# EnyaHermite/SPH3D-GCN

Measured on AMD Instinct MI355X. Metric: point-cloud blocks/sec (fwd+bwd) SPH3D_s3dis 8192-pt, higher is better.
Workload: dtype f32

## Files before the change

### include/sph3d.h

```cpp
#ifndef SPH3D_H
#define SPH3D_H

#include <stddef.h>

#ifdef __cplusplus
extern "C" {
#endif

typedef void* sph3d_stream_t;

enum {
    SPH3D_OK = 0,
    SPH3D_EINVAL = -1,
    SPH3D_EWORKSPACE = -2,
    SPH3D_ELAUNCH = -3,
    SPH3D_EUNSUPPORTED = -4
};

#define SPH3D_ABI_VERSION 2
int sph3d_abi_version(void);
const char* sph3d_last_error(void);
const char* sph3d_build_info(void);


// ... 155 lines not shown
int sph3d_pointwise_gemm_tn(int R, int Cin, int Cout,
                            const float* X, const float* dY, float* dW,
                            void* workspace, size_t workspace_bytes,
                            sph3d_stream_t stream);
size_t sph3d_pointwise_gemm_tn_workspace(int R, int Cin, int Cout);

size_t sph3d_elu_bn_workspace(int R, int C);
int sph3d_elu_bn_forward(int R, int C, const float* y, const float* gamma, const float* beta,
                         float* running_mean, float* running_var, float momentum, float eps, int training,
                         float* out, float* save_mean, float* save_rstd,
                         void* workspace, size_t workspace_bytes, sph3d_stream_t stream);
int sph3d_elu_bn_backward(int R, int C, const float* y, const float* dout, const float* gamma,
                          const float* save_mean, const float* save_rstd, int training,
                          float* dy, float* dgamma, float* dbeta,
                          void* workspace, size_t workspace_bytes, sph3d_stream_t stream);

int sph3d_pointwise_gemm_bnstats_blocks(int R, int Cin, int Cout);
int sph3d_pointwise_gemm_bnstats(int R, int Cin, int Cout, const float* X, const float* W, const float* bias ,
                                 float* Y, float* partial, sph3d_stream_t stream);
int sph3d_elu_bn_forward_partials(int R, int C, int nblk, const float* partial, const float* y, const float* gamma,
                                  const float* beta, float* running_mean, float* running_var, float momentum, float eps,
                                  float* out, float* save_mean, float* save_rstd, sph3d_stream_t stream);

int sph3d_separable_conv3d_fused_supported(int N, int F, int C, int r, int K, int Cout);
int sph3d_separable_conv3d_fused(int B, int N, int M, int F, int C, int r, int K, int Cout, int act,
                                 const int* nn_index, const int* nn_count, const int* bin_index, const float* input,
                                 const float* depthwise_filter, const float* pointwise_weights, const float* bias,
                                 const float* scale, const float* shift, float* output, sph3d_stream_t stream);

int sph3d_separable_conv3d_train_supported(int N, int F, int C, int r, int K, int Cout);
int sph3d_separable_conv3d_train_blocks(int Cout);
int sph3d_separable_conv3d_train(int B, int N, int M, int F, int C, int r, int K, int Cout,
                                 const int* nn_index, const int* nn_count, const int* bin_index, const float* input,
                                 const float* depthwise_filter, const float* pointwise_weights, const float* bias,
                                 float* depthwise_output, float* y, float* partial, sph3d_stream_t stream);
int sph3d_separable_conv3d_ring_failures(void);

int sph3d_pointwise_gemm_skinny_supported(int R, int K1, int K2, int N);
int sph3d_pointwise_gemm_skinny(int R, int K1, int K2, int N, const float* A1, const float* A2, const float* W, const float* bias,
                                float* Y, sph3d_stream_t stream);
size_t sph3d_pointwise_gemm_skinny_tn_workspace(int R, int K1, int K2, int N);
int sph3d_pointwise_gemm_skinny_tn(int R, int K1, int K2, int N, const float* A1, const float* A2, const float* dY, float* dW,
                                   void* workspace, size_t workspace_bytes, sph3d_stream_t stream);

int sph3d_depthwise_conv3d_cat_supported(int F, int Ca, int Cb, int r);
int sph3d_depthwise_conv3d_cat(int B, int N, int M, int F, int Ca, int Cb, int r, int K, const int* nn_index, const int* nn_count,
// ... 24 lines not shown
```

### sph3d_gcn_amd/_lib.py

```python
import ctypes
import os

import torch

_HERE = os.path.dirname(os.path.abspath(__file__))
LIB_PATH = os.environ.get("SPH3D_LIB") or os.path.join(_HERE, "csrc", "libsph3d.so")

_c_int = ctypes.c_int
_c_float = ctypes.c_float
_c_size_t = ctypes.c_size_t
_vp = ctypes.c_void_p

_I, _F, _P, _S = _c_int, _c_float, _vp, _c_size_t
SIGNATURES = {
    "sph3d_abi_version": (_I, []),
    "sph3d_last_error": (ctypes.c_char_p, []),
    "sph3d_build_info": (ctypes.c_char_p, []),
    "sph3d_build_sphere_neighbor": (_I, [_I, _I, _I, _I, _F, _P, _P, _P, _P, _P, _P]),
    "sph3d_build_sphere_neighbor_fixed": (_I, [_I, _I, _I, _I, _F, _P, _P, _P, _P, _P, _P]),
    "sph3d_build_sphere_neighbor_workspace": (_S, [_I, _I, _I]),
    "sph3d_build_sphere_neighbor_ws": (_I, [_I, _I, _I, _I, _F, _P, _P, _P, _P, _P, _P, _S, _P]),
    "sph3d_build_sphere_neighbor_fixed_ws": (_I, [_I, _I, _I, _I, _F, _P, _P, _P, _P, _P, _P, _S, _P]),
    "sph3d_release_stream_scratch": (_I, [_P]),
    "sph3d_release_all_scratch": (_I, []),
# ... 39 lines not shown
    "sph3d_pointwise_gemm_tn": (_I, [_I] * 3 + [_P, _P, _P, _P, _S, _P]),
    "sph3d_elu_bn_workspace": (_S, [_I] * 2),
    "sph3d_pointwise_gemm_bnstats_blocks": (_I, [_I] * 3),
    "sph3d_pointwise_gemm_bnstats": (_I, [_I] * 3 + [_P] * 6),
    "sph3d_nngrid_launches": (ctypes.c_longlong, []),
    "sph3d_masked_softmax_xent_parts": (_I, [_I]),
    "sph3d_masked_softmax_xent": (_I, [_I, _I, _I] + [_P] * 5 + [_P]),
    "sph3d_adam_step": (_I, [ctypes.c_longlong] + [_P] * 4 + [_F] * 4 + [_I, _P]),
    "sph3d_feed_assemble": (_I, [_I, _I, _I, ctypes.c_longlong, _P, _P, _P, ctypes.c_ulonglong, ctypes.c_ulonglong, _I] + [_P] * 5),
    "sph3d_pointwise_gemm_skinny_supported": (_I, [_I] * 4),
    "sph3d_pointwise_gemm_skinny": (_I, [_I] * 4 + [_P] * 6),
    "sph3d_pointwise_gemm_skinny_tn_workspace": (_S, [_I] * 4),
    "sph3d_pointwise_gemm_skinny_tn": (_I, [_I] * 4 + [_P] * 5 + [_S, _P]),
    "sph3d_separable_conv3d_fused_supported": (_I, [_I] * 6),
    "sph3d_separable_conv3d_fused": (_I, [_I] * 9 + [_P] * 11),
    "sph3d_separable_conv3d_train_supported": (_I, [_I] * 6),
    "sph3d_separable_conv3d_train_blocks": (_I, [_I]),
    "sph3d_separable_conv3d_train": (_I, [_I] * 8 + [_P] * 11),
    "sph3d_separable_conv3d_ring_failures": (_I, []),
    "sph3d_pointwise_gemm_exchange_failures": (_I, []),
    "sph3d_elu_bn_forward_partials": (_I, [_I] * 3 + [_P] * 6 + [_F, _F] + [_P] * 4),
    "sph3d_elu_bn_forward": (_I, [_I, _I, _P, _P, _P, _P, _P, _F, _F, _I, _P, _P, _P, _P, _S, _P]),
    "sph3d_elu_bn_backward": (_I, [_I, _I] + [_P] * 5 + [_I] + [_P] * 3 + [_P, _S, _P]),
}
_EXTRA = {
    "sph3d_selftest_math": (_I, [_I, _P, _P, _P, _P, _P, _P, _P]),
}

ABI_VERSION = 2
_lib = None


class Sph3dError(RuntimeError):
    pass


def lib():
    global _lib
    if _lib is not None:
        return _lib
    if not os.path.exists(LIB_PATH):
        raise Sph3dError(
            "libsph3d.so is not built (%s).  Run `python -c 'import __graft_entry__ as g; g.build()'` "
            "or `make -C sph3d_gcn_amd/csrc`.  There is no fallback path." % LIB_PATH)
    l = ctypes.CDLL(LIB_PATH)
    for table in (SIGNATURES, _EXTRA):
# ... 118 lines not shown
def ptr(t):
    return t.data_ptr() if t is not None else None


_scratch = {}


def release_scratch(stream=None):
    for key in [k for k in _scratch if stream is None or k[1] == stream]:
        del _scratch[key]


def scratch(nbytes, device, slot=0):
    if not nbytes:
        return None
    key = (device.index, current_raw_stream(), slot)
    t = _scratch.get(key)
    if t is None or t.numel() < nbytes:
        t = torch.empty((nbytes + nbytes // 4,), dtype=torch.uint8, device=device)
        _scratch[key] = t
    return t


class Arena:
    __slots__ = ("device", "cap", "off", "need", "_i32", "_f32", "buf")

    def __init__(self, nbytes, device):
        self.device, self.cap, self.off, self.need = device, int(nbytes), 0, 0
        self.buf = torch.empty((self.cap,), dtype=torch.uint8, device=device) if self.cap > 0 else None
        self._i32 = self.buf.view(torch.int32) if self.buf is not None else None
        self._f32 = self.buf.view(torch.float32) if self.buf is not None else None

    def take(self, shape, dtype):
        n = 4
        for d in shape:
            n *= d
        n = (n + 255) & ~255
        self.need += n
        if n == 0 or self.buf is None or self.off + n > self.cap:
            return None
        base = self._i32 if dtype is torch.int32 else self._f32
        strides, s = [], 1
        for d in reversed(shape):
            strides.append(s)
            s *= d
        strides.reverse()
# ... 33 lines not shown
```

### sph3d_gcn_amd/csrc/gemm.hip

```cpp
#include <atomic>
#include "common.hpp"

namespace sph3d {

typedef float f32x16 __attribute__((ext_vector_type(16)));
typedef float f32x4 __attribute__((ext_vector_type(4)));
typedef float f32x2 __attribute__((ext_vector_type(2)));
__device__ __forceinline__ f32x4 as_v4(const float4 v) { f32x4 r; r.x = v.x; r.y = v.y; r.z = v.z; r.w = v.w; return r; }

constexpr int BM = 128;
constexpr int BKS = 16;
constexpr int BKL = 32;

__device__ __forceinline__ float4 load4_guard(const float* __restrict__ p, int ld, int r, int c, int rows, int cols, bool vec_ok)
{
    float4 v = make_float4(0.f, 0.f, 0.f, 0.f);
    if (r < rows) {
        const float* q = p + (size_t)r * ld + c;
        if (vec_ok && c + 3 < cols) {
            v = *reinterpret_cast<const float4*>(q);
        } else {
            if (c < cols) v.x = q[0];
            if (c + 1 < cols) v.y = q[1];
            if (c + 2 < cols) v.z = q[2];
// ... 119 lines not shown
    __device__ __forceinline__ void issue(const float* __restrict__ base, float* image) const
    {
        const int wave = __builtin_amdgcn_readfirstlane((int)threadIdx.x >> 6);
#pragma unroll
        for (int i = 0; i < NI; i++) {
            __builtin_amdgcn_global_load_lds((const __attribute__((address_space(1))) void*)(base + voff[i]),
                                             (__attribute__((address_space(3))) void*)(image + (wave * NI + i) * 256), 16, 0, 0);
        }
    }
    static __device__ __forceinline__ f32x4 frag(const float* image, int row, int g, int lk)
    {
        if (KM) return *reinterpret_cast<const f32x4*>(image + ((row << 2) + ((2 * g + lk) ^ ((row >> 2) & 3))) * 4);
        const float* q = image + (8 * g + 4 * lk) * BT + (row ^ (lk << 5));
        return f32x4{q[0], q[BT], q[2 * BT], q[3 * BT]};
    }
};

constexpr int kDmaWgs = 5;
constexpr int cmax_i(int a, int b) { return a > b ? a : b; }

template <int BMT, int BN, int TM, int TN, bool SPLITK, bool GUARD, bool STATS, bool EPX, int LDSF>
__device__ __forceinline__ void gemm_epilogue(f32x16 (&acc)[TM][TN], float* lds, int M, int N, float* __restrict__ Cmat, int ldc,
                                              const float* __restrict__ bias, int act, float* __restrict__ stats, int tm, int ksplit,
                                              int m0, int n0, int wave, int lane, int wm, int wn, int li, int lk)
{
    constexpr int WN = BN / 2;
    float* Cout = SPLITK ? Cmat + (size_t)ksplit * ((size_t)M * ldc) : Cmat;
    if (!GUARD) {
        constexpr int EP = EPX ? WN : WN + 4;
        static_assert(4 * 32 * EP <= LDSF, "epilogue staging must fit the operand LDS");
        float* stage = lds + wave * (32 * EP);
        constexpr int LPR = WN / 4;
        constexpr int RPI = 64 / LPR;
        if constexpr (STATS) {
#pragma unroll
            for (int j = 0; j < TN; j++) {
                const float bv = bias != nullptr ? bias[n0 + wn + j * 32 + li] : 0.f;
                float sz = 0.f, sq = 0.f;
#pragma unroll
                for (int i = 0; i < TM; i++)
#pragma unroll
                    for (int e = 0; e < 16; e++) {
                        const float y = acc[i][j][e] + bv;
                        const float z = y > 0.f ? y : __expf(y) - 1.f;
                        sz += z;
                        sq = fmaf(z, z, sq);
                    }
                sz += __shfl_xor(sz, 32);
                sq += __shfl_xor(sq, 32);
                if (lk == 0) {
                    float* sp = stats + (size_t)(tm * 2 + (wave >> 1)) * 2 * N + n0 + wn + j * 32 + li;
                    sp[0] = sz;
                    sp[N] = sq;
                }
            }
        }
#pragma unroll
        for (int i = 0; i < TM; i++) {
#pragma unroll
            for (int j = 0; j < TN; j++) {
                const int col = wn + j * 32 + li;
                const float bv = (!SPLITK && bias != nullptr) ? bias[n0 + col] : 0.f;
#pragma unroll
                for (int e = 0; e < 16; e++) {
                    float v = acc[i][j][e] + bv;
                    if (!SPLITK && act == 1) v = v > 0.f ? v : expm1f(v);
                    stage[((e & 3) + 8 * (e >> 2) + 4 * lk) * EP + ((j * 32 + li) ^ (EPX ? (lk << 5) : 0))] = v;
                }
            }
#pragma unroll
            for (int it = 0; it < 32 / RPI; it++) {
                const int r = it * RPI + lane / LPR;
                const int c4 = (lane % LPR) * 4;
                const float4 v = *reinterpret_cast<const float4*>(&stage[r * EP + (c4 ^ (EPX ? (((r >> 2) & 1) << 5) : 0))]);
                *reinterpret_cast<float4*>(&Cout[(size_t)(m0 + wm + i * 32 + r) * ldc + n0 + wn + c4]) = v;
            }
        }
        return;
    }
#pragma unroll
    for (int i = 0; i < TM; i++) {
#pragma unroll
        for (int j = 0; j < TN; j++) {
            const int col = n0 + wn + j * 32 + li;
            const float bv = (!SPLITK && bias != nullptr && col < N) ? bias[col] : 0.f;
#pragma unroll
            for (int e = 0; e < 16; e++) {
                const int row = m0 + wm + i * 32 + (e & 3) + 8 * (e >> 2) + 4 * lk;
                if (row < M && col < N) {
                    float v = acc[i][j][e] + bv;
                    if (!SPLITK && act == 1) v = v > 0.f ? v : expm1f(v);
                    Cout[(size_t)row * ldc + col] = v;
                }
            }
        }
    }
}

template <bool AK, bool BKM, int BMT, int BN, int BK, bool SPLITK, bool GUARD, bool STATS = false>
__global__ __launch_bounds__(256, (BK == 16 && !GUARD) ? kDmaWgs : 2) void gemm_f32_mfma(int M, int N, int Kd, const float* __restrict__ A, int lda,
                                                     const float* __restrict__ B, int ldb, float* __restrict__ Cmat,
                                                     int ldc, const float* __restrict__ bias, int act, int kchunk,
                                                     float* __restrict__ stats = nullptr, int nsplit = 1)
{
    using SA = Stage<AK, BMT, BK>;
    using SB = Stage<BKM, BN, BK>;
    constexpr int LDK = BK + 4;
    constexpr bool DMA = !GUARD && BK == 16;
    constexpr int WM = BMT / 2, WN = BN / 2;
    constexpr int LDSF = DMA ? cmax_i(2 * (BMT + BN) * BK, 4 * 32 * (WN == 64 ? WN : WN + 4)) : 2 * (SA::LDS_FLOATS + SB::LDS_FLOATS);
    __shared__ __attribute__((aligned(16))) float lds[LDSF];
    constexpr int TM = WM / 32, TN = WN / 32;

    const int tiles_n = (N + BN - 1) / BN;
    const int tiles_m = (M + BMT - 1) / BMT;
    const int wg = (int)blockIdx.x;
    int tm, tn, ksplit = 0;
    if (SPLITK) {
        const int T = tiles_m * tiles_n;
        const int g = wg / (8 * T), r = wg - g * 8 * T;
        ksplit = g * 8 + (r & 7);
        if (ksplit >= nsplit) return;
        const int tile = r >> 3;
        tm = tile / tiles_n;
        tn = tile - tm * tiles_n;
    } else {
// ... 119 lines not shown
            for (int s4 = 0; s4 < 4; s4++) {
#pragma unroll
                for (int i = 0; i < TM; i++)
#pragma unroll
                    for (int j = 0; j < TN; j++) {
                        const float av = s4 == 0 ? af[i].x : (s4 == 1 ? af[i].y : (s4 == 2 ? af[i].z : af[i].w));
                        const float bv = s4 == 0 ? bf[j].x : (s4 == 1 ? bf[j].y : (s4 == 2 ? bf[j].z : bf[j].w));
                        acc[i][j] = __builtin_amdgcn_mfma_f32_32x32x2f32(av, bv, acc[i][j], 0, 0, 0);
                    }
            }
        }
        __builtin_amdgcn_s_setprio(0);
        if (more) {
            sa.store(lds + (buf ^ 1) * BUF);
            sb.store(lds + (buf ^ 1) * BUF + SA::LDS_FLOATS);
        }
        __syncthreads();
        buf ^= 1;
    }

    }

    gemm_epilogue<BMT, BN, TM, TN, SPLITK, GUARD, STATS, DMA && WN == 64, LDSF>(acc, lds, M, N, Cmat, ldc, bias, act, stats, tm, ksplit,
                                                                                  m0, n0, wave, lane, wm, wn, li, lk);
}

typedef __bf16 bf16x8 __attribute__((ext_vector_type(8)));
typedef unsigned u32x2v __attribute__((ext_vector_type(2)));

struct Split3 { unsigned h, m, l; };
__device__ __forceinline__ Split3 split_pair(float a, float b)
{
    Split3 r;
    const unsigned ua = __float_as_uint(a), ub = __float_as_uint(b);
    r.h = __builtin_amdgcn_perm(ub, ua, 0x07060302u);
    const float ra = a - __uint_as_float(ua & 0xffff0000u), rb = b - __uint_as_float(ub & 0xffff0000u);
    const unsigned va = __float_as_uint(ra), vb = __float_as_uint(rb);
    r.m = __builtin_amdgcn_perm(vb, va, 0x07060302u);
    const float sa = ra - __uint_as_float(va & 0xffff0000u), sb = rb - __uint_as_float(vb & 0xffff0000u);
    r.l = __builtin_amdgcn_perm(__float_as_uint(sb), __float_as_uint(sa), 0x07060302u);
    return r;
}

template <bool KMAJ, int BT, int BK>
struct SplitStage {
    static constexpr int KG = BK / 8;
    static constexpr int PLANE = KG * BT * 16;
// ... 65 lines not shown
                for (int j = 0; j < 4; j++) {
                    const Split3 sp = split_pair(a[j], b[j]);
                    char* q = img + (slot(k0 >> 3, rq * 4 + j) << 4) + ((k0 & 7) << 1);
                    *reinterpret_cast<unsigned*>(q) = sp.h;
                    *reinterpret_cast<unsigned*>(q + PLANE) = sp.m;
                    *reinterpret_cast<unsigned*>(q + 2 * PLANE) = sp.l;
                }
            }
        }
    }
    __device__ __forceinline__ static bf16x8 frag(const char* img, int pc, int row, int g)
    {
        return *reinterpret_cast<const bf16x8*>(img + pc * PLANE + (slot(g, row) << 4));
    }
};

__device__ int g_xs_fail = 0;

template <bool AK, bool BKM, int BMT, int BN, int BK, bool SPLITK, bool STATS, bool GUARD = false, bool XS = false>
__global__ __launch_bounds__(256, 4) void gemm_split_mfma(int M, int N, int Kd, const float* __restrict__ A, int lda,
                                                          const float* __restrict__ B, int ldb, float* __restrict__ Cmat, int ldc,
                                                          const float* __restrict__ bias, int act, int kchunk,
                                                          float* __restrict__ stats = nullptr, int nsplit = 1,
                                                          float* __restrict__ xslab = nullptr, int* __restrict__ xflag = nullptr)
{
    static_assert(!(XS && SPLITK) && !(XS && GUARD), "the exchange variant is an unguarded, non-slab kernel");
    using PA = SplitStage<AK, BMT, BK>;
    using PB = SplitStage<BKM, BN, BK>;
    constexpr int WM = BMT / 2, WN = BN / 2;
    constexpr int TM = WM / 32, TN = WN / 32;
    constexpr int BUFB = PA::BYTES + PB::BYTES;
    constexpr bool EPX = WN == 64;
    constexpr int LDSF = cmax_i(BUFB / 4, 4 * 32 * (EPX ? WN : WN + 4));
    __shared__ __attribute__((aligned(16))) float lds[LDSF];
    char* img = reinterpret_cast<char*>(lds);

    const int tiles_n = (N + BN - 1) / BN;
    const int tiles_m = (M + BMT - 1) / BMT;
    const int wg = (int)blockIdx.x;
    int tm, tn, ksplit = 0;
    if (XS) {
        const int Tg = ((tiles_m + 7) / 8) * 8 * tiles_n;
        const int rev = wg / Tg, wl = wg - rev * Tg;
        ksplit = nsplit - 1 - rev;
        const int g = wl / (8 * tiles_n), r = wl - g * 8 * tiles_n;
        tm = g * 8 + (r & 7);
        tn = r >> 3;
// ... 115 lines not shown
            int polls = 0;
            while (__hip_atomic_load(&xflag[tile], __ATOMIC_RELAXED, __HIP_MEMORY_SCOPE_AGENT) < nsplit - 1) {
                __builtin_amdgcn_s_sleep(4);
                if (++polls > (1 << 20)) {
                    atomicAdd(&g_xs_fail, 1);
                    break;
                }
            }
            __hip_atomic_store(&xflag[tile], 0, __ATOMIC_RELAXED, __HIP_MEMORY_SCOPE_AGENT);
        }
        __syncthreads();
        for (int ks = 1; ks < nsplit; ks++) {
            const float* sl = xslab + ((size_t)(ks - 1) * ntile + tile) * (NW * 256) + threadIdx.x;
#pragma unroll
            for (int i = 0; i < TM; i++)
#pragma unroll
                for (int j = 0; j < TN; j++)
#pragma unroll
                    for (int e = 0; e < 16; e++)
                        acc[i][j][e] += __hip_atomic_load(&sl[((i * TN + j) * 16 + e) * 256], __ATOMIC_RELAXED, __HIP_MEMORY_SCOPE_AGENT);
        }
    }
    gemm_epilogue<BMT, BN, TM, TN, SPLITK, GUARD, STATS, EPX, LDSF>(acc, lds, M, N, Cmat, ldc, bias, act, stats, tm, ksplit, m0, n0, wave,
                                                                      lane, wm, wn, li, lk);
}

__global__ __launch_bounds__(256) void gemm_reduce_splits(int nsplit, int total, const float* __restrict__ partial,
                                                          float* __restrict__ out)
{
    __shared__ float red[8][32];
    const int cx = (int)threadIdx.x & 31, py = (int)threadIdx.x >> 5;
    const int j = blockIdx.x * 32 + cx;
    float s = 0.f;
    if (j < total) {
        for (int p0 = py; p0 < nsplit; p0 += 64) {
            float v[8];
#pragma unroll
            for (int u = 0; u < 8; u++) {
                const int p = p0 + u * 8;
                v[u] = partial[(size_t)(p < nsplit ? p : py) * total + j];
            }
#pragma unroll
            for (int u = 0; u < 8; u++)
                if (p0 + u * 8 < nsplit) s += v[u];
        }
    }
    red[py][cx] = s;
// ... 144 lines not shown
extern "C" int sph3d_pointwise_gemm_mode(int mode)
{
    if (mode == 0 || mode == 1) return g_split_mode.exchange(mode);
    return g_split_mode.load();
}

extern "C" int sph3d_pointwise_gemm(int R, int Cin, int Cout, const float* X, const float* W, const float* bias, int act,
                                    int trans_w, float* Y, sph3d_stream_t stream)
{
    SPH3D_REQUIRE(R >= 0 && Cin > 0 && Cout > 0, "pointwise_gemm: bad dims R=%d Cin=%d Cout=%d", R, Cin, Cout);
    SPH3D_REQUIRE(act == 0 || act == 1, "pointwise_gemm: act must be 0 (none) or 1 (ELU), got %d", act);
    if (R == 0) return SPH3D_OK;
    hipStream_t st = as_stream(stream);
    if (trans_w) return launch_gemm<true, true>(R, Cout, Cin, X, Cin, W, Cin, Y, Cout, bias, act, st);
    return launch_gemm<true, false>(R, Cout, Cin, X, Cin, W, Cout, Y, Cout, bias, act, st);
}

extern "C" int sph3d_pointwise_gemm_bnstats_blocks(int R, int Cin, int Cout)
{
    int bm = 0, bn = 0;
    return (R > 0 && Cin > 0 && Cout > 0) ? nn_stats_tile(R, Cout, Cin, bm, bn) : 0;
}

extern "C" int sph3d_pointwise_gemm_bnstats(int R, int Cin, int Cout, const float* X, const float* W, const float* bias, float* Y,
                                            float* partial, sph3d_stream_t stream)
{
    SPH3D_REQUIRE(R > 0 && Cin > 0 && Cout > 0, "pointwise_gemm_bnstats: bad dims R=%d Cin=%d Cout=%d", R, Cin, Cout);
    int bm = 0, bn = 0;
    const int nblk = nn_stats_tile(R, Cout, Cin, bm, bn);
    if (nblk == 0 || !aligned16(X) || !aligned16(W) || !aligned16(Y)) {
        set_error("pointwise_gemm_bnstats: shape (%d, %d -> %d) needs whole tiles and 16-byte aligned operands", R, Cin, Cout);
        return SPH3D_EUNSUPPORTED;
    }
    hipStream_t st = as_stream(stream);
    const unsigned tiles = gemm_grid(R / bm, Cout / bn);
    if (split_on()) {
        if (bm == 128 && bn == 128)
            hipLaunchKernelGGL((gemm_split_mfma<true, false, 128, 128, 16, false, true>), dim3(tiles), dim3(256), 0, st, R, Cout, Cin, X, Cin, W,
                               Cout, Y, Cout, bias, 0, 0, partial);
        else if (bm == 128)
            hipLaunchKernelGGL((gemm_split_mfma<true, false, 128, 64, 16, false, true>), dim3(tiles), dim3(256), 0, st, R, Cout, Cin, X, Cin, W,
                               Cout, Y, Cout, bias, 0, 0, partial);
        else if (Cin % 32 == 0) {
            const int ns = xs_splits(tiles, Cin, 32, kXsCap);
            char* xb = ns > 1 ? xs_buffer(st, (long long)(R / 64) * (Cout / 64), ns, 64 * 64) : nullptr;
            if (xb != nullptr)
                hipLaunchKernelGGL((gemm_split_mfma<true, false, 64, 64, 32, false, true, false, true>), dim3(tiles * ns), dim3(256), 0, st, R, Cout,
                                   Cin, X, Cin, W, Cout, Y, Cout, bias, 0, Cin / ns, partial, ns, (float*)(xb + kXsFlagBytes), (int*)xb);
            else
                hipLaunchKernelGGL((gemm_split_mfma<true, false, 64, 64, 32, false, true>), dim3(tiles), dim3(256), 0, st, R, Cout, Cin, X, Cin, W,
                                   Cout, Y, Cout, bias, 0, 0, partial);
        } else
            hipLaunchKernelGGL((gemm_split_mfma<true, false, 64, 64, 16, false, true>), dim3(tiles), dim3(256), 0, st, R, Cout, Cin, X, Cin, W,
                               Cout, Y, Cout, bias, 0, 0, partial);
        return check_launch("sph3d_pointwise_gemm_bnstats");
    }
    if (bm == 128 && bn == 128)
        hipLaunchKernelGGL((gemm_f32_mfma<true, false, 128, 128, BKS, false, false, true>), dim3(tiles), dim3(256), 0, st, R, Cout, Cin, X,
                           Cin, W, Cout, Y, Cout, bias, 0, 0, partial);
    else if (bm == 128)
        hipLaunchKernelGGL((gemm_f32_mfma<true, false, 128, 64, BKS, false, false, true>), dim3(tiles), dim3(256), 0, st, R, Cout, Cin, X,
                           Cin, W, Cout, Y, Cout, bias, 0, 0, partial);
    else
        hipLaunchKernelGGL((gemm_f32_mfma<true, false, 64, 64, BKS, false, false, true>), dim3(tiles), dim3(256), 0, st, R, Cout, Cin, X,
                           Cin, W, Cout, Y, Cout, bias, 0, 0, partial);
    return check_launch("sph3d_pointwise_gemm_bnstats");
}

extern "C" size_t sph3d_pointwise_gemm_tn_workspace(int R, int Cin, int Cout)
{
    int bn, tiles, nsplit, kchunk;
    tn_plan(R, Cin, Cout, bn, tiles, nsplit, kchunk);
    return nsplit > 1 ? sizeof(float) * (size_t)nsplit * Cin * Cout : 0;
}

extern "C" int sph3d_pointwise_gemm_tn(int R, int Cin, int Cout, const float* X, const float* dY, float* dW,
                                       void* workspace, size_t workspace_bytes, sph3d_stream_t stream)
{
    SPH3D_REQUIRE(R > 0 && Cin > 0 && Cout > 0, "pointwise_gemm_tn: bad dims R=%d Cin=%d Cout=%d", R, Cin, Cout);
    hipStream_t st = as_stream(stream);
    int bn, tiles, nsplit, kchunk;
    tn_plan(R, Cin, Cout, bn, tiles, nsplit, kchunk);
    const size_t need = sph3d_pointwise_gemm_tn_workspace(R, Cin, Cout);
    if (need > 0 && (workspace == nullptr || workspace_bytes < need)) {
        set_error("pointwise_gemm_tn: workspace %zu B < required %zu B", workspace_bytes, need);
        return SPH3D_EWORKSPACE;
    }
    float* out = nsplit > 1 ? (float*)workspace : dW;
    const bool whole = (Cin % 128 == 0) && (Cout % bn == 0) && (R % kchunk == 0) && aligned16(X) && aligned16(dY) && aligned16(out);
// ... 44 lines not shown
```

### sph3d_gcn_amd/csrc/norm.hip

```cpp
#include "common.hpp"

namespace sph3d {

constexpr int kNormMaxBlocks = 1024;

__device__ __forceinline__ float elu1(float y) { return y > 0.f ? y : __expf(y) - 1.f; }

template <bool BWD>
__global__ __launch_bounds__(256) void norm_reduce_kernel(int R, int C, const float* __restrict__ y,
                                                          const float* __restrict__ dout, const float* __restrict__ mean,
                                                          const float* __restrict__ rstd, float* __restrict__ partial)
{
    __shared__ float4 red[2][256];
    const int cg = C >> 2;
    const int rows_per_iter = 256 / cg > 0 ? 256 / cg : 1;
    const int tx = (int)threadIdx.x % cg, ty = (int)threadIdx.x / cg;
    const bool act = ty < rows_per_iter;
    const int rows_per_block = (R + (int)gridDim.x - 1) / (int)gridDim.x;
    const int r0 = (int)blockIdx.x * rows_per_block;
    const int r1 = (r0 + rows_per_block) < R ? (r0 + rows_per_block) : R;
    float4 a = make_float4(0.f, 0.f, 0.f, 0.f), b = a;
    float4 mu = a, rs = a;
    if (BWD && act) {
        mu = *reinterpret_cast<const float4*>(&mean[tx * 4]);
// ... 146 lines not shown
            o.y = fmaf((elu1(v.y) - mu.y) * rs.y, ga.y, be.y);
            o.z = fmaf((elu1(v.z) - mu.z) * rs.z, ga.z, be.z);
            o.w = fmaf((elu1(v.w) - mu.w) * rs.w, ga.w, be.w);
        } else {
            const float4 g = reinterpret_cast<const float4*>(dout)[i];
            const float4 c0 = *reinterpret_cast<const float4*>(&coef[c]);
            const float4 c1 = *reinterpret_cast<const float4*>(&coef[C + c]);
#define SPH3D_BN_BWD(e)                                                             \
    {                                                                               \
        const float z = elu1(v.e);                                                  \
        const float zh = (z - mu.e) * rs.e;                                         \
        const float dz = ga.e * rs.e * (g.e - c0.e - zh * c1.e);                    \
        o.e = v.e > 0.f ? dz : dz * (z + 1.f);                                      \
    }
            SPH3D_BN_BWD(x) SPH3D_BN_BWD(y) SPH3D_BN_BWD(z) SPH3D_BN_BWD(w)
#undef SPH3D_BN_BWD
        }
        reinterpret_cast<float4*>(out)[i] = o;
    }
}

static int norm_blocks(int R) { int b = (R + 31) / 32; return b < 1 ? 1 : (b > kNormMaxBlocks ? kNormMaxBlocks : b); }

}

using namespace sph3d;

extern "C" size_t sph3d_elu_bn_workspace(int R, int C)
{
    return sizeof(float) * ((size_t)norm_blocks(R) * 2 * C + 2 * (size_t)C);
}

extern "C" int sph3d_elu_bn_forward(int R, int C, const float* y, const float* gamma, const float* beta,
                                    float* running_mean, float* running_var, float momentum, float eps, int training,
                                    float* out, float* save_mean, float* save_rstd,
                                    void* workspace, size_t workspace_bytes, sph3d_stream_t stream)
{
    SPH3D_REQUIRE(R > 0 && C > 0 && C % 4 == 0 && C <= 1024, "elu_bn: needs R>0, C%%4==0, C<=1024 (got R=%d C=%d)", R, C);
    const size_t need = sph3d_elu_bn_workspace(R, C);
    if (workspace == nullptr || workspace_bytes < need) {
        set_error("elu_bn_forward: workspace %zu B < required %zu B", workspace_bytes, need);
        return SPH3D_EWORKSPACE;
    }
    hipStream_t st = as_stream(stream);
    float* partial = (float*)workspace;
    const int nblk = norm_blocks(R);
// ... 35 lines not shown
                                     const float* save_mean, const float* save_rstd, int training,
                                     float* dy, float* dgamma, float* dbeta,
                                     void* workspace, size_t workspace_bytes, sph3d_stream_t stream)
{
    SPH3D_REQUIRE(R > 0 && C > 0 && C % 4 == 0 && C <= 1024, "elu_bn: needs R>0, C%%4==0, C<=1024 (got R=%d C=%d)", R, C);
    const size_t need = sph3d_elu_bn_workspace(R, C);
    if (workspace == nullptr || workspace_bytes < need) {
        set_error("elu_bn_backward: workspace %zu B < required %zu B", workspace_bytes, need);
        return SPH3D_EWORKSPACE;
    }
    hipStream_t st = as_stream(stream);
    float* partial = (float*)workspace;
    const int nblk = norm_blocks(R);
    float* coef = partial + (size_t)nblk * 2 * C;
    hipLaunchKernelGGL(norm_reduce_kernel<true>, dim3(nblk), dim3(256), 0, st, R, C, y, dout, save_mean, save_rstd, partial);
    hipLaunchKernelGGL(norm_bwd_finalize, dim3((C + 31) / 32), dim3(32 * kFinLanes), 0, st, R, C, nblk, training, partial, dgamma, dbeta, coef);
    const long long total4 = (long long)R * C / 4;
    long long blocks = (total4 + 255) / 256;
    if (blocks > 4096) blocks = 4096;
    hipLaunchKernelGGL(norm_apply_kernel<true>, dim3((unsigned)blocks), dim3(256), 0, st, total4, C, y, dout, save_mean,
                       save_rstd, gamma, nullptr, coef, dy);
    return check_launch("sph3d_elu_bn_backward");
}
```

### sph3d_gcn_amd/tf_norm.py

```python
from typing import Optional, Tuple

import torch

from . import _lib

MOMENTUM = 0.99
EPSILON = 1e-3


def supported(C):
    return C % 4 == 0 and C <= 1024


def _fwd_impl(y: torch.Tensor, gamma: torch.Tensor, beta: torch.Tensor, moving_mean: torch.Tensor,
              moving_var: torch.Tensor, training: bool) -> Tuple[torch.Tensor, torch.Tensor, torch.Tensor]:
    _lib.require_device(y, gamma, beta, moving_mean, moving_var)
    y = _lib.f32(y)
    C = y.shape[-1]
    R = y.numel() // C
    out = torch.empty_like(y)
    save_mean = torch.empty((C,), dtype=torch.float32, device=y.device)
    save_rstd = torch.empty((C,), dtype=torch.float32, device=y.device)
    l = _lib.lib()
    wsb = l.sph3d_elu_bn_workspace(R, C)
# ... 89 lines not shown
    save_rstd = torch.empty((C,), dtype=torch.float32, device=y.device)
    _lib.check(_lib.lib().sph3d_elu_bn_forward_partials(R, C, partial.shape[0], _lib.ptr(partial), _lib.ptr(y), _lib.ptr(gamma),
                                                         _lib.ptr(beta), _lib.ptr(moving_mean), _lib.ptr(moving_var),
                                                         1.0 - MOMENTUM, EPSILON, _lib.ptr(out), _lib.ptr(save_mean),
                                                         _lib.ptr(save_rstd), _lib.stream_ptr()))
    return out, save_mean, save_rstd


_gemm_bnstats = torch.library.custom_op("sph3d::pointwise_gemm_bnstats", mutates_args=())(_gemm_bnstats_impl)
_elu_bn_partials = torch.library.custom_op("sph3d::elu_bn_partials", mutates_args=("moving_mean", "moving_var"))(_elu_bn_partials_impl)


@_gemm_bnstats.register_fake
def _(x, w, bias=None):
    nblk = gemm_bn_blocks(x.shape[0], x.shape[1], w.shape[1])
    return x.new_empty((x.shape[0], w.shape[1])), x.new_empty((nblk, 2, w.shape[1]))


@_elu_bn_partials.register_fake
def _(y, partial, gamma, beta, moving_mean, moving_var):
    return torch.empty_like(y), torch.empty_like(gamma), torch.empty_like(gamma)


class _GemmEluBnFn(torch.autograd.Function):

    @staticmethod
    def forward(ctx, x, w, bias, gamma, beta, moving_mean, moving_var):
        y, partial = _gemm_bnstats_impl(x, w, bias)
        out, save_mean, save_rstd = _elu_bn_partials_impl(y, partial, gamma, beta, moving_mean, moving_var)
        ctx.save_for_backward(x, w, y, gamma, save_mean, save_rstd)
        ctx.has_bias = bias is not None
        return out

    @staticmethod
    def backward(ctx, dout):
        from . import tf_gemm
        x, w, y, gamma, save_mean, save_rstd = ctx.saved_tensors
        dy, dgamma, dbeta = _bwd_impl(y, dout, gamma, save_mean, save_rstd, True)
        dx = tf_gemm._pointwise_gemm_impl(dy, w, True) if ctx.needs_input_grad[0] else None
        dw = tf_gemm._pointwise_gemm_tn_impl(x, dy) if ctx.needs_input_grad[1] else None
        db = dy.sum(0) if (ctx.has_bias and ctx.needs_input_grad[2]) else None
        return dx, dw, db, dgamma, dbeta, None, None


def gemm_elu_batch_norm(x, w, gamma, beta, moving_mean, moving_var, bias=None):
    return _GemmEluBnFn.apply(x, w, bias, gamma, beta, moving_mean, moving_var)
```

Baseline: 2059.

## Fold batch-norm statistics finalize into GEMM tail via last-block reduction

Adds a last-arriving-workgroup tail to the pointwise GEMM+BN-stats kernel. Workgroups count arrivals with atomic counters, the final block of each row group reduces the per-tile partials in double, and a final group computes mean, rstd and the running stats. This removes the separate stats-reduction pass that the old partials-based forward launched. The apply step is now a lightweight separate kernel. In exchange it adds atomic counters, persistent zeroed scratch and a serialized tail inside the GEMM, with a fallback launch when there are few blocks.

```diff
diff --git a/include/sph3d.h b/include/sph3d.h
--- a/include/sph3d.h
+++ b/include/sph3d.h
@@ -201,6 +201,15 @@
                                   const float* beta, float* running_mean, float* running_var, float momentum, float eps,
                                   float* out, float* save_mean, float* save_rstd, sph3d_stream_t stream);
 
+size_t sph3d_pointwise_gemm_bnstats_tail_workspace(int R, int Cin, int Cout);
+size_t sph3d_pointwise_gemm_bnstats_tail_counters_workspace(void);
+int sph3d_pointwise_gemm_bnstats_tail(int R, int Cin, int Cout, const float* X, const float* W, const float* bias ,
+                                      float* Y, float* running_mean, float* running_var, float momentum, float eps,
+                                      float* save_mean, float* save_rstd, void* workspace, size_t workspace_bytes,
+                                      void* counters, sph3d_stream_t stream);
+int sph3d_elu_bn_apply(int R, int C, const float* y, const float* gamma, const float* beta, const float* save_mean,
+                       const float* save_rstd, float* out, sph3d_stream_t stream);
+
 int sph3d_separable_conv3d_fused_supported(int N, int F, int C, int r, int K, int Cout);
 int sph3d_separable_conv3d_fused(int B, int N, int M, int F, int C, int r, int K, int Cout, int act,
                                  const int* nn_index, const int* nn_count, const int* bin_index, const float* input,
diff --git a/sph3d_gcn_amd/_lib.py b/sph3d_gcn_amd/_lib.py
--- a/sph3d_gcn_amd/_lib.py
+++ b/sph3d_gcn_amd/_lib.py
@@ -85,6 +85,10 @@
     "sph3d_elu_bn_forward_partials": (_I, [_I] * 3 + [_P] * 6 + [_F, _F] + [_P] * 4),
     "sph3d_elu_bn_forward": (_I, [_I, _I, _P, _P, _P, _P, _P, _F, _F, _I, _P, _P, _P, _P, _S, _P]),
     "sph3d_elu_bn_backward": (_I, [_I, _I] + [_P] * 5 + [_I] + [_P] * 3 + [_P, _S, _P]),
+    "sph3d_pointwise_gemm_bnstats_tail_counters_workspace": (_S, []),
+    "sph3d_elu_bn_apply": (_I, [_I, _I] + [_P] * 7),
+    "sph3d_pointwise_gemm_bnstats_tail_workspace": (_S, [_I] * 3),
+    "sph3d_pointwise_gemm_bnstats_tail": (_I, [_I] * 3 + [_P] * 6 + [_F, _F] + [_P] * 3 + [_S, _P, _P]),
 }
 _EXTRA = {
     "sph3d_selftest_math": (_I, [_I, _P, _P, _P, _P, _P, _P, _P]),
@@ -249,6 +253,15 @@
     return t
 
 
+def zeroed_scratch(nbytes, device, slot):
+    key = (device.index, current_raw_stream(), slot)
+    t = _scratch.get(key)
+    if t is None or t.numel() < nbytes:
+        t = torch.zeros((nbytes,), dtype=torch.uint8, device=device)
+        _scratch[key] = t
+    return t
+
+
 class Arena:
     __slots__ = ("device", "cap", "off", "need", "_i32", "_f32", "buf")
 
diff --git a/sph3d_gcn_amd/csrc/bn_tail.hpp b/sph3d_gcn_amd/csrc/bn_tail.hpp
--- /dev/null
+++ b/sph3d_gcn_amd/csrc/bn_tail.hpp
@@ -0,0 +1,140 @@
+#pragma once
+#include <hip/hip_runtime.h>
+
+namespace sph3d {
+
+constexpr int kBnTailMaxGroups = 64;
+constexpr int kBnTailCounterWords = 128;
+constexpr int kBnTailLdsBytes = 16 + 2 * 256 * 8;
+
+struct BnTail {
+    unsigned* cnt = nullptr;
+    double* gsum = nullptr;
+    int rpg = 0;
+    int R = 0;
+    float* o0 = nullptr;
+    float* o1 = nullptr;
+    float* o2 = nullptr;
+    float* o3 = nullptr;
+    float eps = 0.f, momentum = 0.f;
+    int training = 1;
+};
+
+constexpr int kBnTailMinRows = 1024;
+void launch_norm_fwd_finalize(int R, int C, int nblk, const float* partial, float eps, float momentum, float* mean, float* rstd,
+                              float* run_mean, float* run_var, hipStream_t st);
+
+static inline int bn_tail_rows_per_group(int nrows)
+{
+    if (nrows <= 64) return nrows;
+    const int need = ((nrows + kBnTailMaxGroups - 1) / kBnTailMaxGroups + 1) & ~1;
+    return need > 32 ? need : 32;
+}
+static inline int bn_tail_groups(int nrows) { const int g = bn_tail_rows_per_group(nrows); return (nrows + g - 1) / g; }
+
+__device__ __forceinline__ void bn_tail_store(float* p, float v) { __hip_atomic_store(p, v, __ATOMIC_RELAXED, __HIP_MEMORY_SCOPE_AGENT); }
+
+__device__ __forceinline__ bool bn_tail_last(unsigned* cnt, unsigned expect, unsigned* flag)
+{
+    asm volatile("s_waitcnt vmcnt(0)" ::: "memory");
+    __syncthreads();
+    if (threadIdx.x == 0) {
+        const unsigned t = __hip_atomic_fetch_add(cnt, 1u, __ATOMIC_RELAXED, __HIP_MEMORY_SCOPE_AGENT);
+        const bool last = t == expect - 1;
+        if (last) __hip_atomic_store(cnt, 0u, __ATOMIC_RELAXED, __HIP_MEMORY_SCOPE_AGENT);
+        *flag = last ? 1u : 0u;
+    }
+    __syncthreads();
+    const bool last = *flag != 0u;
+    __builtin_amdgcn_fence(__ATOMIC_ACQUIRE, "wavefront");
+    return last;
+}
+
+template <typename T>
+__device__ __forceinline__ void bn_tail_fold(const T* src, int C, int k0, int k1, int cb, double* red, double& s, double& q, bool& own)
+{
+    const int tid = (int)threadIdx.x;
+    const int P = C >= 256 ? 1 : 256 / C;
+    const int c = cb + (C >= 256 ? tid : tid % C);
+    const int p = C >= 256 ? 0 : tid / C;
+    const bool act = c < C && p < P;
+    s = 0.0; q = 0.0;
+    if (act) {
+        constexpr int UN = 8;
+        for (int kb = k0 + p; kb < k1; kb += UN * P) {
+            T a[UN], b[UN];
+#pragma unroll
+            for (int u = 0; u < UN; u++) {
+                const int k = kb + u * P;
+                const int kc = k < k1 ? k : kb;
+                a[u] = __hip_atomic_load(&src[(size_t)kc * 2 * C + c], __ATOMIC_RELAXED, __HIP_MEMORY_SCOPE_AGENT);
+                b[u] = __hip_atomic_load(&src[(size_t)kc * 2 * C + C + c], __ATOMIC_RELAXED, __HIP_MEMORY_SCOPE_AGENT);
+            }
+#pragma unroll
+            for (int u = 0; u < UN; u++)
+                if (kb + u * P < k1) { s += (double)a[u]; q += (double)b[u]; }
+        }
+    }
+    red[tid] = s;
+    red[256 + tid] = q;
+    __syncthreads();
+    own = act && p == 0;
+    if (own)
+        for (int j = 1; j < P; j++) { s += red[j * C + (c - cb)]; q += red[256 + j * C + (c - cb)]; }
+    __syncthreads();
+}
+
+template <bool BWD>
+__device__ __forceinline__ void bn_tail_outputs(const BnTail& t, int C, int c, double s, double q)
+{
+    if (!BWD) {
+        const double m = s / t.R;
+        double var = q / t.R - m * m;
+        if (var < 0.0) var = 0.0;
+        t.o0[c] = (float)m;
+        t.o1[c] = (float)(1.0 / sqrt(var + (double)t.eps));
+        if (t.o2 != nullptr) {
+            t.o2[c] = (float)((1.0 - t.momentum) * t.o2[c] + t.momentum * m);
+            t.o3[c] = (float)((1.0 - t.momentum) * t.o3[c] + t.momentum * var);
+        }
+    } else {
+        t.o0[c] = (float)s;
+        t.o1[c] = (float)q;
+        t.o2[c] = t.training ? (float)(s / t.R) : 0.f;
+        t.o2[C + c] = t.training ? (float)(q / t.R) : 0.f;
+    }
+}
+
+template <bool BWD>
+__device__ __forceinline__ void bn_tail_finish(const BnTail& t, const float* partial, int C, int nrows, int group, int arrivals, void* lds)
+{
+    unsigned* flag = reinterpret_cast<unsigned*>(lds);
+    double* red = reinterpret_cast<double*>(reinterpret_cast<char*>(lds) + 16);
+    if (!bn_tail_last(&t.cnt[1 + group], (unsigned)arrivals, flag)) return;
+    const int ngroups = (nrows + t.rpg - 1) / t.rpg;
+    const int k0 = group * t.rpg;
+    const int k1 = (k0 + t.rpg) < nrows ? (k0 + t.rpg) : nrows;
+    for (int cb = 0; cb < C; cb += 256) {
+        double s, q;
+        bool own;
+        bn_tail_fold<float>(partial, C, k0, k1, cb, red, s, q, own);
+        if (own) {
+            const int c = cb + (C >= 256 ? (int)threadIdx.x : (int)threadIdx.x % C);
+            if (ngroups == 1) bn_tail_outputs<BWD>(t, C, c, s, q);
+            else {
+                __hip_atomic_store(&t.gsum[(size_t)group * 2 * C + c], s, __ATOMIC_RELAXED, __HIP_MEMORY_SCOPE_AGENT);
+                __hip_atomic_store(&t.gsum[(size_t)group * 2 * C + C + c], q, __ATOMIC_RELAXED, __HIP_MEMORY_SCOPE_AGENT);
+            }
+        }
+    }
+    if (ngroups == 1) return;
+    if (!bn_tail_last(&t.cnt[0], (unsigned)ngroups, flag)) return;
+    for (int cb = 0; cb < C; cb += 256) {
+        double s, q;
+        bool own;
+        bn_tail_fold<double>(t.gsum, C, 0, ngroups, cb, red, s, q, own);
+        if (own) bn_tail_outputs<BWD>(t, C, cb + (C >= 256 ? (int)threadIdx.x : (int)threadIdx.x % C), s, q);
+    }
+}
+
+}
diff --git a/sph3d_gcn_amd/csrc/gemm.hip b/sph3d_gcn_amd/csrc/gemm.hip
--- a/sph3d_gcn_amd/csrc/gemm.hip
+++ b/sph3d_gcn_amd/csrc/gemm.hip
@@ -1,5 +1,6 @@
 #include <atomic>
 #include "common.hpp"
+#include "bn_tail.hpp"
 
 namespace sph3d {
 
@@ -165,7 +166,7 @@
 template <int BMT, int BN, int TM, int TN, bool SPLITK, bool GUARD, bool STATS, bool EPX, int LDSF>
 __device__ __forceinline__ void gemm_epilogue(f32x16 (&acc)[TM][TN], float* lds, int M, int N, float* __restrict__ Cmat, int ldc,
                                               const float* __restrict__ bias, int act, float* __restrict__ stats, int tm, int ksplit,
-                                              int m0, int n0, int wave, int lane, int wm, int wn, int li, int lk)
+                                              int m0, int n0, int wave, int lane, int wm, int wn, int li, int lk, const BnTail& fin)
 {
     constexpr int WN = BN / 2;
     float* Cout = SPLITK ? Cmat + (size_t)ksplit * ((size_t)M * ldc) : Cmat;
@@ -193,8 +194,13 @@
                 sq += __shfl_xor(sq, 32);
                 if (lk == 0) {
                     float* sp = stats + (size_t)(tm * 2 + (wave >> 1)) * 2 * N + n0 + wn + j * 32 + li;
-                    sp[0] = sz;
-                    sp[N] = sq;
+                    if (fin.cnt == nullptr) {
+                        sp[0] = sz;
+                        sp[N] = sq;
+                    } else {
+                        bn_tail_store(sp, sz);
+                        bn_tail_store(sp + N, sq);
+                    }
                 }
             }
         }
@@ -217,6 +223,15 @@
                 const int c4 = (lane % LPR) * 4;
                 const float4 v = *reinterpret_cast<const float4*>(&stage[r * EP + (c4 ^ (EPX ? (((r >> 2) & 1) << 5) : 0))]);
                 *reinterpret_cast<float4*>(&Cout[(size_t)(m0 + wm + i * 32 + r) * ldc + n0 + wn + c4]) = v;
+            }
+        }
+        if constexpr (STATS) {
+            if (fin.cnt != nullptr) {
+                static_assert(LDSF * 4 >= kBnTailLdsBytes, "the finish borrows the operand LDS");
+                const int tiles_m = M / BMT, tiles_n = N / BN;
+                const int tpg = fin.rpg >> 1, group = tm / tpg;
+                const int t1 = (group + 1) * tpg < tiles_m ? (group + 1) * tpg : tiles_m;
+                bn_tail_finish<false>(fin, stats, N, 2 * tiles_m, group, (t1 - group * tpg) * tiles_n, lds);
             }
         }
         return;
@@ -244,7 +259,7 @@
 __global__ __launch_bounds__(256, (BK == 16 && !GUARD) ? kDmaWgs : 2) void gemm_f32_mfma(int M, int N, int Kd, const float* __restrict__ A, int lda,
                                                      const float* __restrict__ B, int ldb, float* __restrict__ Cmat,
                                                      int ldc, const float* __restrict__ bias, int act, int kchunk,
-                                                     float* __restrict__ stats = nullptr, int nsplit = 1)
+                                                     float* __restrict__ stats = nullptr, int nsplit = 1, BnTail fin = {})
 {
     using SA = Stage<AK, BMT, BK>;
     using SB = Stage<BKM, BN, BK>;
@@ -410,7 +425,7 @@
     }
 
     gemm_epilogue<BMT, BN, TM, TN, SPLITK, GUARD, STATS, DMA && WN == 64, LDSF>(acc, lds, M, N, Cmat, ldc, bias, act, stats, tm, ksplit,
-                                                                                  m0, n0, wave, lane, wm, wn, li, lk);
+                                                                                  m0, n0, wave, lane, wm, wn, li, lk, fin);
 }
 
 typedef __bf16 bf16x8 __attribute__((ext_vector_type(8)));
@@ -522,7 +537,8 @@
                                                           const float* __restrict__ B, int ldb, float* __restrict__ Cmat, int ldc,
                                                           const float* __restrict__ bias, int act, int kchunk,
                                                           float* __restrict__ stats = nullptr, int nsplit = 1,
-                                                          float* __restrict__ xslab = nullptr, int* __restrict__ xflag = nullptr)
+                                                          float* __restrict__ xslab = nullptr, int* __restrict__ xflag = nullptr,
+                                                          BnTail fin = {})
 {
     static_assert(!(XS && SPLITK) && !(XS && GUARD), "the exchange variant is an unguarded, non-slab kernel");
     using PA = SplitStage<AK, BMT, BK>;
@@ -684,7 +700,7 @@
         }
     }
     gemm_epilogue<BMT, BN, TM, TN, SPLITK, GUARD, STATS, EPX, LDSF>(acc, lds, M, N, Cmat, ldc, bias, act, stats, tm, ksplit, m0, n0, wave,
-                                                                      lane, wm, wn, li, lk);
+                                                                      lane, wm, wn, li, lk, fin);
 }
 
 __global__ __launch_bounds__(256) void gemm_reduce_splits(int nsplit, int total, const float* __restrict__ partial,
@@ -875,49 +891,96 @@
     return (R > 0 && Cin > 0 && Cout > 0) ? nn_stats_tile(R, Cout, Cin, bm, bn) : 0;
 }
 
-extern "C" int sph3d_pointwise_gemm_bnstats(int R, int Cin, int Cout, const float* X, const float* W, const float* bias, float* Y,
-                                            float* partial, sph3d_stream_t stream)
-{
-    SPH3D_REQUIRE(R > 0 && Cin > 0 && Cout > 0, "pointwise_gemm_bnstats: bad dims R=%d Cin=%d Cout=%d", R, Cin, Cout);
+static int launch_bnstats(const char* what, int R, int Cin, int Cout, const float* X, const float* W, const float* bias, float* Y,
+                          float* partial, BnTail fin, hipStream_t st)
+{
     int bm = 0, bn = 0;
     const int nblk = nn_stats_tile(R, Cout, Cin, bm, bn);
     if (nblk == 0 || !aligned16(X) || !aligned16(W) || !aligned16(Y)) {
-        set_error("pointwise_gemm_bnstats: shape (%d, %d -> %d) needs whole tiles and 16-byte aligned operands", R, Cin, Cout);
+        set_error("%s: shape (%d, %d -> %d) needs whole tiles and 16-byte aligned operands", what, R, Cin, Cout);
         return SPH3D_EUNSUPPORTED;
     }
-    hipStream_t st = as_stream(stream);
+    float* const nof = nullptr;
+    int* const noi = nullptr;
     const unsigned tiles = gemm_grid(R / bm, Cout / bn);
     if (split_on()) {
         if (bm == 128 && bn == 128)
             hipLaunchKernelGGL((gemm_split_mfma<true, false, 128, 128, 16, false, true>), dim3(tiles), dim3(256), 0, st, R, Cout, Cin, X, Cin, W,
-                               Cout, Y, Cout, bias, 0, 0, partial);
+                               Cout, Y, Cout, bias, 0, 0, partial, 1, nof, noi, fin);
         else if (bm == 128)
             hipLaunchKernelGGL((gemm_split_mfma<true, false, 128, 64, 16, false, true>), dim3(tiles), dim3(256), 0, st, R, Cout, Cin, X, Cin, W,
-                               Cout, Y, Cout, bias, 0, 0, partial);
+                               Cout, Y, Cout, bias, 0, 0, partial, 1, nof, noi, fin);
         else if (Cin % 32 == 0) {
             const int ns = xs_splits(tiles, Cin, 32, kXsCap);
             char* xb = ns > 1 ? xs_buffer(st, (long long)(R / 64) * (Cout / 64), ns, 64 * 64) : nullptr;
             if (xb != nullptr)
                 hipLaunchKernelGGL((gemm_split_mfma<true, false, 64, 64, 32, false, true, false, true>), dim3(tiles * ns), dim3(256), 0, st, R, Cout,
-                                   Cin, X, Cin, W, Cout, Y, Cout, bias, 0, Cin / ns, partial, ns, (float*)(xb + kXsFlagBytes), (int*)xb);
+                                   Cin, X, Cin, W, Cout, Y, Cout, bias, 0, Cin / ns, partial, ns, (float*)(xb + kXsFlagBytes), (int*)xb, fin);
             else
                 hipLaunchKernelGGL((gemm_split_mfma<true, false, 64, 64, 32, false, true>), dim3(tiles), dim3(256), 0, st, R, Cout, Cin, X, Cin, W,
-                                   Cout, Y, Cout, bias, 0, 0, partial);
+                                   Cout, Y, Cout, bias, 0, 0, partial, 1, nof, noi, fin);
         } else
             hipLaunchKernelGGL((gemm_split_mfma<true, false, 64, 64, 16, false, true>), dim3(tiles), dim3(256), 0, st, R, Cout, Cin, X, Cin, W,
-                               Cout, Y, Cout, bias, 0, 0, partial);
-        return check_launch("sph3d_pointwise_gemm_bnstats");
+                               Cout, Y, Cout, bias, 0, 0, partial, 1, nof, noi, fin);
+        return check_launch(what);
     }
     if (bm == 128 && bn == 128)
         hipLaunchKernelGGL((gemm_f32_mfma<true, false, 128, 128, BKS, false, false, true>), dim3(tiles), dim3(256), 0, st, R, Cout, Cin, X,
-                           Cin, W, Cout, Y, Cout, bias, 0, 0, partial);
+                           Cin, W, Cout, Y, Cout, bias, 0, 0, partial, 1, fin);
     else if (bm == 128)
         hipLaunchKernelGGL((gemm_f32_mfma<true, false, 128, 64, BKS, false, false, true>), dim3(tiles), dim3(256), 0, st, R, Cout, Cin, X,
-                           Cin, W, Cout, Y, Cout, bias, 0, 0, partial);
+                           Cin, W, Cout, Y, Cout, bias, 0, 0, partial, 1, fin);
     else
         hipLaunchKernelGGL((gemm_f32_mfma<true, false, 64, 64, BKS, false, false, true>), dim3(tiles), dim3(256), 0, st, R, Cout, Cin, X,
-                           Cin, W, Cout, Y, Cout, bias, 0, 0, partial);
-    return check_launch("sph3d_pointwise_gemm_bnstats");
+                           Cin, W, Cout, Y, Cout, bias, 0, 0, partial, 1, fin);
+    return check_launch(what);
+}
+
+extern "C" int sph3d_pointwise_gemm_bnstats(int R, int Cin, int Cout, const float* X, const float* W, const float* bias, float* Y,
+                                            float* partial, sph3d_stream_t stream)
+{
+    SPH3D_REQUIRE(R > 0 && Cin > 0 && Cout > 0, "pointwise_gemm_bnstats: bad dims R=%d Cin=%d Cout=%d", R, Cin, Cout);
+    return launch_bnstats("sph3d_pointwise_gemm_bnstats", R, Cin, Cout, X, W, bias, Y, partial, BnTail{}, as_stream(stream));
+}
+
+static size_t bnstats_partial_bytes(int nblk, int Cout) { return (sizeof(float) * (size_t)nblk * 2 * Cout + 7) & ~(size_t)7; }
+
+extern "C" size_t sph3d_pointwise_gemm_bnstats_tail_workspace(int R, int Cin, int Cout)
+{
+    const int nblk = sph3d_pointwise_gemm_bnstats_blocks(R, Cin, Cout);
+    if (nblk == 0) return 0;
+    return bnstats_partial_bytes(nblk, Cout) + sizeof(double) * (size_t)bn_tail_groups(nblk) * 2 * Cout;
+}
+
+extern "C" size_t sph3d_pointwise_gemm_bnstats_tail_counters_workspace(void) { return sizeof(unsigned) * kBnTailCounterWords; }
+
+extern "C" int sph3d_pointwise_gemm_bnstats_tail(int R, int Cin, int Cout, const float* X, const float* W, const float* bias, float* Y,
+                                                 float* running_mean, float* running_var, float momentum, float eps,
+                                                 float* save_mean, float* save_rstd, void* workspace, size_t workspace_bytes,
+                                                 void* counters, sph3d_stream_t stream)
+{
+    SPH3D_REQUIRE(R > 0 && Cin > 0 && Cout > 0 && Cout <= 1024, "pointwise_gemm_bnstats_tail: bad dims R=%d Cin=%d Cout=%d", R, Cin, Cout);
+    const int nblk = sph3d_pointwise_gemm_bnstats_blocks(R, Cin, Cout);
+    const size_t need = sph3d_pointwise_gemm_bnstats_tail_workspace(R, Cin, Cout);
+    if (nblk > 0 && (workspace == nullptr || workspace_bytes < need || counters == nullptr)) {
+        set_error("pointwise_gemm_bnstats_tail: workspace %zu B < required %zu B, or no counters", workspace_bytes, need);
+        return SPH3D_EWORKSPACE;
+    }
+    hipStream_t st = as_stream(stream);
+    if (nblk < kBnTailMinRows) {
+        const int rc = launch_bnstats("sph3d_pointwise_gemm_bnstats_tail", R, Cin, Cout, X, W, bias, Y, (float*)workspace, BnTail{}, st);
+        if (rc != SPH3D_OK) return rc;
+        launch_norm_fwd_finalize(R, Cout, nblk, (const float*)workspace, eps, momentum, save_mean, save_rstd, running_mean, running_var, st);
+        return check_launch("sph3d_pointwise_gemm_bnstats_tail");
+    }
+    BnTail t;
+    t.cnt = (unsigned*)counters;
+    t.gsum = (double*)((char*)workspace + bnstats_partial_bytes(nblk, Cout));
+    t.rpg = bn_tail_rows_per_group(nblk);
+    t.R = R;
+    t.o0 = save_mean; t.o1 = save_rstd; t.o2 = running_mean; t.o3 = running_var;
+    t.eps = eps; t.momentum = momentum;
+    return launch_bnstats("sph3d_pointwise_gemm_bnstats_tail", R, Cin, Cout, X, W, bias, Y, (float*)workspace, t, st);
 }
 
 extern "C" size_t sph3d_pointwise_gemm_tn_workspace(int R, int Cin, int Cout)
diff --git a/sph3d_gcn_amd/csrc/norm.hip b/sph3d_gcn_amd/csrc/norm.hip
--- a/sph3d_gcn_amd/csrc/norm.hip
+++ b/sph3d_gcn_amd/csrc/norm.hip
@@ -1,4 +1,5 @@
 #include "common.hpp"
+#include "bn_tail.hpp"
 
 namespace sph3d {
 
@@ -192,6 +193,13 @@
 
 static int norm_blocks(int R) { int b = (R + 31) / 32; return b < 1 ? 1 : (b > kNormMaxBlocks ? kNormMaxBlocks : b); }
 
+void launch_norm_fwd_finalize(int R, int C, int nblk, const float* partial, float eps, float momentum, float* mean, float* rstd,
+                              float* run_mean, float* run_var, hipStream_t st)
+{
+    hipLaunchKernelGGL(norm_fwd_finalize, dim3((C + 31) / 32), dim3(32 * kFinLanes), 0, st, R, C, nblk, partial, eps, momentum, mean, rstd,
+                       run_mean, run_var);
+}
+
 }
 
 using namespace sph3d;
@@ -273,3 +281,15 @@
                        save_rstd, gamma, nullptr, coef, dy);
     return check_launch("sph3d_elu_bn_backward");
 }
+
+extern "C" int sph3d_elu_bn_apply(int R, int C, const float* y, const float* gamma, const float* beta, const float* save_mean,
+                                  const float* save_rstd, float* out, sph3d_stream_t stream)
+{
+    SPH3D_REQUIRE(R > 0 && C > 0 && C % 4 == 0 && C <= 1024, "elu_bn_apply: needs R>0, C%%4==0, C<=1024 (got R=%d C=%d)", R, C);
+    const long long total4 = (long long)R * C / 4;
+    long long blocks = (total4 + 255) / 256;
+    if (blocks > 4096) blocks = 4096;
+    hipLaunchKernelGGL(norm_apply_kernel<false>, dim3((unsigned)blocks), dim3(256), 0, as_stream(stream), total4, C, y, nullptr, save_mean,
+                       save_rstd, gamma, beta, nullptr, out);
+    return check_launch("sph3d_elu_bn_apply");
+}
diff --git a/sph3d_gcn_amd/tf_norm.py b/sph3d_gcn_amd/tf_norm.py
--- a/sph3d_gcn_amd/tf_norm.py
+++ b/sph3d_gcn_amd/tf_norm.py
@@ -135,12 +135,40 @@
     return torch.empty_like(y), torch.empty_like(gamma), torch.empty_like(gamma)
 
 
+def _counters(device):
+    return _lib.zeroed_scratch(_lib.lib().sph3d_pointwise_gemm_bnstats_tail_counters_workspace(), device, "bn_tail_counters")
+
+
+def _gemm_bnstats_tail_impl(x, w, bias, gamma, beta, moving_mean, moving_var):
+    _lib.require_device(x, w, gamma, beta, moving_mean, moving_var)
+    x, w = _lib.f32(x), _lib.f32(w)
+    if bias is not None:
+        bias = _lib.f32(bias)
+    R, Cin = x.shape
+    Cout = w.shape[1]
+    l = _lib.lib()
+    wsb = l.sph3d_pointwise_gemm_bnstats_tail_workspace(R, Cin, Cout)
+    if wsb == 0:
+        raise ValueError("pointwise_gemm_bnstats: shape (%d, %d -> %d) is not covered (whole tiles needed)" % (R, Cin, Cout))
+    ws = _lib.scratch(wsb, x.device)
+    y = torch.empty((R, Cout), dtype=torch.float32, device=x.device)
+    out = torch.empty_like(y)
+    save_mean = torch.empty((Cout,), dtype=torch.float32, device=x.device)
+    save_rstd = torch.empty((Cout,), dtype=torch.float32, device=x.device)
+    _lib.check(l.sph3d_pointwise_gemm_bnstats_tail(R, Cin, Cout, _lib.ptr(x), _lib.ptr(w), _lib.ptr(bias), _lib.ptr(y),
+                                                   _lib.ptr(moving_mean), _lib.ptr(moving_var), 1.0 - MOMENTUM, EPSILON,
+                                                   _lib.ptr(save_mean), _lib.ptr(save_rstd), _lib.ptr(ws), wsb,
+                                                   _lib.ptr(_counters(x.device)), _lib.stream_ptr()))
+    _lib.check(l.sph3d_elu_bn_apply(R, Cout, _lib.ptr(y), _lib.ptr(gamma), _lib.ptr(beta), _lib.ptr(save_mean),
+                                    _lib.ptr(save_rstd), _lib.ptr(out), _lib.stream_ptr()))
+    return y, out, save_mean, save_rstd
+
+
 class _GemmEluBnFn(torch.autograd.Function):
 
     @staticmethod
     def forward(ctx, x, w, bias, gamma, beta, moving_mean, moving_var):
-        y, partial = _gemm_bnstats_impl(x, w, bias)
-        out, save_mean, save_rstd = _elu_bn_partials_impl(y, partial, gamma, beta, moving_mean, moving_var)
+        y, out, save_mean, save_rstd = _gemm_bnstats_tail_impl(x, w, bias, gamma, beta, moving_mean, moving_var)
         ctx.save_for_backward(x, w, y, gamma, save_mean, save_rstd)
         ctx.has_bias = bias is not None
         return out
```

Result: no change. 2069, median of 6 (+0.5%).
